# yunminjin2/KD-PointCloud

Measured on AMD Instinct MI355X. Metric: scene-flow pairs/sec fwd+bwd @ N=8192; EPE3D vs ref; 1/2/4/8 MI355X, higher is better.
Workload: dtype f32; 1 GPU; PointConvBidirection fwd+bwd+Adam (BASELINE configs[2]); model=models_bid_pointconv.PointConvBidirection, batch_per_gpu=8, global_batch=8, npoints=8192, parallelism=dp1, step=hip-graph (1 graph: fwd+bwd+flat Adam)

## Files before the change

### kd-pointcloud_amd/csrc/cost_volume.hip

```cpp
#include <algorithm>

#include "kdpc_common.h"
#include "split_bf16.h"

using namespace kdpc;
using namespace kdpc_x6;

namespace {

typedef float f32x16 __attribute__((ext_vector_type(16)));
typedef float f32x4 __attribute__((ext_vector_type(4)));

constexpr float kSlope = 0.1f;
constexpr int kRows = 32;
constexpr int kWaves = 4;

__device__ __forceinline__ float lrelu(float x) { return x > 0.f ? x : x * kSlope; }

__device__ __forceinline__ float bload(__amdgpu_buffer_rsrc_t r, unsigned off) {
  return __builtin_bit_cast(float, __builtin_amdgcn_raw_buffer_load_b32(r, (int)off, 0, 0));
}
__device__ __forceinline__ __amdgpu_buffer_rsrc_t rsrc_of(const void* p, long long bytes) {
  return __builtin_amdgcn_make_buffer_rsrc(const_cast<void*>(p), (short)0, (int)bytes, 0x00020000);
}
// ... 223 lines not shown
    bwp[ks] = split8(v);
  }
  const float w0 = wpos[cg * 3 + 0], wy = wpos[cg * 3 + 1], wz = wpos[cg * 3 + 2], bp = bpos[cg];

  const float* x1b = x1 + (long long)b * n1 * 3;
  const __amdgpu_buffer_rsrc_t x2r = rsrc_of(x2 + (long long)b * n2 * 3, (long long)n2 * 12);
  const __amdgpu_buffer_rsrc_t ixr = rsrc_of(idx + (long long)b * n1 * k, (long long)n1 * k * 4);
  const __amdgpu_buffer_rsrc_t p1r = rsrc_of(p1 + (long long)b * n1 * D_IN, (long long)n1 * D_IN * 4);
  const __amdgpu_buffer_rsrc_t p2r = rsrc_of(p2 + (long long)b * n2 * D_IN, (long long)n2 * D_IN * 4);
  const long long ob0 = (long long)b * n1 * D_OUT;
  const __amdgpu_buffer_rsrc_t outr = rsrc_of(out + ob0, (long long)n1 * D_OUT * 4);
  const __amdgpu_buffer_rsrc_t dor = rsrc_of(dout + ob0, (long long)n1 * D_OUT * 4);
  const __amdgpu_buffer_rsrc_t amr = rsrc_of(amax + ob0, (long long)n1 * D_OUT);
  const __amdgpu_buffer_rsrc_t s0r =
      rsrc_of(OVR ? slope0 + (long long)b * n1 * k * D_IN : amax, OVR ? (long long)n1 * k * D_IN : 0);
  const bool ranked = rank != nullptr;
  const __amdgpu_buffer_rsrc_t rkr = rsrc_of(ranked ? rank + (long long)b * n1 * k : idx,
                                             ranked ? (long long)n1 * k * 4 : 0);
  const long long nrow_all = (long long)nb * n1 * k;
  const __amdgpu_buffer_rsrc_t rowr = rsrc_of(rows_out, rows_out ? nrow_all * D_IN * 4 : 0);
  const __amdgpu_buffer_rsrc_t dirr = rsrc_of(dirs_out, dirs_out ? nrow_all * (ranked ? 16 : 12) : 0);
  const int nbase = b * n1;

  float gw1[DW1_MFMA ? 1 : D_OUT / 2];
  f32x16 gw[DW1_MFMA ? OT : 1];
  if constexpr (DW1_MFMA) {
#pragma unroll
    for (int t = 0; t < OT; ++t) gw[t] = f32x16{0};
  } else {
#pragma unroll
    for (int i = 0; i < D_OUT / 2; ++i) gw1[i] = 0.f;
  }
  float gb1[OT];
#pragma unroll
  for (int t = 0; t < OT; ++t) gb1[t] = 0.f;
  float gpx[2] = {0.f, 0.f}, gpy[2] = {0.f, 0.f}, gpz[2] = {0.f, 0.f};
  float gbp = 0.f;

  const int q0 = (bx * (kWaves / CS) + qw) * queries_per_wave;
  const int q1 = min(n1, q0 + queries_per_wave);
  int jn = (int)__builtin_amdgcn_raw_buffer_load_b32(ixr, (int)(((unsigned)q0 * (unsigned)k + lane) * 4u), 0, 0);
  float pv[8][2];
  float xv0, xv1, xv2, p1v, ovq[OT], dvq[OT];
  float qs0, qs1, qs2;
  auto load_q = [&](int n) {
    const int nq = min(n, n1 - 1);
    qs0 = x1b[nq * 3 + 0];
    qs1 = x1b[nq * 3 + 1];
    qs2 = x1b[nq * 3 + 2];
  };
  int amq[OT], rkn;
  auto load_idx = [&](int n) {
    jn = (int)__builtin_amdgcn_raw_buffer_load_b32(ixr, (int)(((unsigned)n * (unsigned)k + lane) * 4u), 0, 0);
  };
  auto issue = [&](int n) {
    const unsigned xo = (unsigned)jn * 12u;
    xv0 = bload(x2r, xo);
    xv1 = bload(x2r, xo + 4u);
    xv2 = bload(x2r, xo + 8u);
#pragma unroll
    for (int t = 0; t < OT; ++t) {
      const unsigned oo = (unsigned)n * D_OUT + 32 * t + l32;
      ovq[t] = bload(outr, oo * 4u);
      dvq[t] = bload(dor, oo * 4u);
      amq[t] = (int)__builtin_amdgcn_raw_buffer_load_b8(amr, (int)oo, 0, 0);
    }
    rkn = (int)__builtin_amdgcn_raw_buffer_load_b32(
        rkr, (int)(lane < k ? ((unsigned)n * (unsigned)k + lane) * 4u : kOOB), 0, 0);
    jT[lane] = jn;
    wave_lds_sync();
    load_idx(n + 1);
#pragma unroll
    for (int q = 0; q < 4; ++q) {
      const int4 j4 = *reinterpret_cast<const int4*>(jT + 8 * q + 4 * half);
      pv[2 * q][0] = bload(p2r, ((unsigned)j4.x * D_IN + cg) * 4u);
      pv[2 * q][1] = bload(p2r, ((unsigned)j4.y * D_IN + cg) * 4u);
      pv[2 * q + 1][0] = bload(p2r, ((unsigned)j4.z * D_IN + cg) * 4u);
      pv[2 * q + 1][1] = bload(p2r, ((unsigned)j4.w * D_IN + cg) * 4u);
    }
    p1v = bload(p1r, ((unsigned)n * D_IN + cg) * 4u);
  };
  float gqn[OT];
  int amn[OT], rkm = -1;
  auto tables = [&](int m, int u) {
#pragma unroll
    for (int t = 0; t < OT; ++t) {
      gqn[t] = dvq[t] * (ovq[t] > 0.f ? 1.f : kSlope);
      amn[t] = amq[t];
    }
    rkm = rkn;
    const int slot = lane < k ? (ranked ? rkm : (nbase + m) * k + lane) : -1;
    float* x = dX(u);
    x[lane] = xv0 - qs0;
    x[2 * kRows + lane] = xv1 - qs1;
    x[4 * kRows + lane] = xv2 - qs2;
    dO(u)[lane] = slot >= 0 ? (unsigned)slot * (unsigned)(D_IN * 4) : kOOB;
#pragma unroll
    for (int t = 0; t < OT; ++t) {
      gdam(u)[32 * t + l32] = make_float2(gqn[t], __int_as_float(amn[t]));
      __bf16 gh, gm, gl;
      split3(gqn[t], gh, gm, gl);
      gpl(u)[32 * t + l32] = gh;
      gpl(u)[D_OUT + 32 * t + l32] = gm;
      gpl(u)[2 * D_OUT + 32 * t + l32] = gl;
      g16(u)[32 * t + l32] = (unsigned short)amn[t];
    }
  };
  float h0[8][2];
  auto build_h0 = [&](int u) {
    const float* x = dX(u);
#pragma unroll
    for (int q = 0; q < 4; ++q) {
      const f32x4 X4 = *reinterpret_cast<const f32x4*>(x + 8 * q + 4 * half);
      const f32x4 Y4 = *reinterpret_cast<const f32x4*>(x + 2 * kRows + 8 * q + 4 * half);
      const f32x4 Z4 = *reinterpret_cast<const f32x4*>(x + 4 * kRows + 8 * q + 4 * half);
#pragma unroll
      for (int e = 0; e < 4; ++e) {
        const float pos = __fadd_rn(
            __builtin_fmaf(wz, Z4[e], __builtin_fmaf(wy, Y4[e], __fmul_rn(w0, X4[e]))), bp);
        const float z = __fadd_rn(__fadd_rn(pv[2 * q + (e >> 1)][e & 1], p1v), pos);
        h0[2 * q + (e >> 1)][e & 1] = fmaxf(z, __fmul_rn(z, kSlope));
      }
      __builtin_amdgcn_sched_barrier(0);
    }
  };
  issue(q0);
  load_q(q0);
  tables(q0, 0);
  load_q(q0 + 1);
  wave_lds_sync();
  build_h0(0);
  const int nit = CS > 1 ? queries_per_wave : q1 - q0;
  for (int it = 0; it < nit; ++it) {
    const int n = q0 + it;
    const int cu = it & 1;
    const bool act = CS == 1 || n < q1;
    float g0 = 0.f, g1 = 0.f, g2 = 0.f;
    const int rkv = rkm;
    float gq[OT];
    int amc[OT];
#pragma unroll
    for (int t = 0; t < OT; ++t) {
      gq[t] = gqn[t];
      amc[t] = amn[t];
    }
    if (act) {
      const float* xc = dX(cu);
      const unsigned* oc = dO(cu);
      const __bf16* gp = gpl(cu);
      const unsigned short* ga16 = g16(cu);
      wave_lds_sync();
      if constexpr (!DW1_MFMA) {
#pragma unroll
        for (int e = 0; e < 16; ++e) T[((e & 3) + 8 * (e >> 2) + 4 * half) * LD + l32] = h0[e >> 1][e & 1];
      }
      __builtin_amdgcn_sched_barrier(0);
      issue(n + 1);
      __builtin_amdgcn_sched_barrier(0);
      f32x16 dacc = f32x16{0};
      {
        typedef short s16x2 __attribute__((ext_vector_type(2)));
        const unsigned tgt = (unsigned)l32 * 0x00010001u;
#pragma unroll
        for (int ks = 0; ks < NKS; ++ks) {
          const int o0 = 16 * ks + 8 * half;
          const uint4 av4 = *reinterpret_cast<const uint4*>(ga16 + o0);
          const uint4 ph = *reinterpret_cast<const uint4*>(gp + o0);
          const uint4 pm = *reinterpret_cast<const uint4*>(gp + D_OUT + o0);
          const uint4 pq = *reinterpret_cast<const uint4*>(gp + 2 * D_OUT + o0);
          const unsigned aw[4] = {av4.x, av4.y, av4.z, av4.w};
          unsigned mk[4];
#pragma unroll
          for (int i = 0; i < 4; ++i) {
            const s16x2 d = __builtin_bit_cast(s16x2, aw[i] ^ tgt) - (s16x2){1, 1};
            mk[i] = __builtin_bit_cast(unsigned, d >> (s16x2){15, 15});
          }
          const uint4 mh = make_uint4(ph.x & mk[0], ph.y & mk[1], ph.z & mk[2], ph.w & mk[3]);
          const uint4 mm = make_uint4(pm.x & mk[0], pm.y & mk[1], pm.z & mk[2], pm.w & mk[3]);
          const uint4 ml = make_uint4(pq.x & mk[0], pq.y & mk[1], pq.z & mk[2], pq.w & mk[3]);
          dacc = mfma_x6(__builtin_bit_cast(bf16x8, mh), __builtin_bit_cast(bf16x8, mm),
                         __builtin_bit_cast(bf16x8, ml), bwp[ks].h, bwp[ks].m, bwp[ks].l, dacc);
          __builtin_amdgcn_sched_barrier(0);
        }
      }
      if constexpr (DW1_MFMA) {
        Planes hp[2];
#pragma unroll
        for (int ks2 = 0; ks2 < 2; ++ks2) {
          float v[8];
#pragma unroll
          for (int j = 0; j < 8; ++j) v[j] = h0[4 * ks2 + (j >> 1)][j & 1];
          hp[ks2] = split8(v);
        }
#pragma unroll
        for (int t = 0; t < OT; ++t) {
          const int am = amc[t];
          const bool mine = ((am >> 2) & 1) == half;
          const int e = (am & 3) + 4 * (am >> 3);
          __bf16 gh, gm, gl;
          split3(gq[t], gh, gm, gl);
          const unsigned sh = (e & 1) * 16;
          const unsigned bh = (unsigned)__builtin_bit_cast(unsigned short, gh) << sh;
          const unsigned bm = (unsigned)__builtin_bit_cast(unsigned short, gm) << sh;
          const unsigned bl = (unsigned)__builtin_bit_cast(unsigned short, gl) << sh;
#pragma unroll
          for (int ks2 = 0; ks2 < 2; ++ks2) {
            unsigned wh[4], wm[4], wl[4];
#pragma unroll
            for (int d = 0; d < 4; ++d) {
              const bool sel = mine && (e >> 1) == 4 * ks2 + d;
              wh[d] = sel ? bh : 0u;
              wm[d] = sel ? bm : 0u;
              wl[d] = sel ? bl : 0u;
            }
            gw[t] = mfma_x6(__builtin_bit_cast(bf16x8, make_uint4(wh[0], wh[1], wh[2], wh[3])),
                            __builtin_bit_cast(bf16x8, make_uint4(wm[0], wm[1], wm[2], wm[3])),
                            __builtin_bit_cast(bf16x8, make_uint4(wl[0], wl[1], wl[2], wl[3])),
                            hp[ks2].h, hp[ks2].m, hp[ks2].l, gw[t]);
          }
          __builtin_amdgcn_sched_barrier(0);
        }
// ... 10 lines not shown
      wave_lds_sync();
      __builtin_amdgcn_sched_barrier(0);
      float dz[8][2];
#pragma unroll
      for (int i = 0; i < 8; ++i) {
#pragma unroll
        for (int p = 0; p < 2; ++p) {
          const float d2 = dacc[2 * i + p];
          bool pass = h0[i][p] > 0.f;
          if constexpr (OVR) {
            const int e = 2 * i + p, r = (e & 3) + 8 * (e >> 2) + 4 * half;
            const unsigned o = __builtin_amdgcn_raw_buffer_load_b8(
                s0r, (int)((((unsigned)n * (unsigned)k + r) * D_IN + cg)), 0, 0);
            pass = o == 1u ? true : (o == 2u ? false : pass);
          }
          dz[i][p] = pass ? d2 : __fmul_rn(d2, kSlope);
        }
      }
      __builtin_amdgcn_sched_barrier(0);
      tables(n + 1, cu ^ 1);
      load_q(n + 2);
      __builtin_amdgcn_sched_barrier(0);
      float dpp1[2] = {0.f, 0.f};
      const unsigned cgo = (unsigned)cg * 4u;
#pragma unroll
      for (int q = 0; q < 4; ++q) {
        const uint4 O4 = *reinterpret_cast<const uint4*>(oc + 8 * q + 4 * half);
        const f32x4 X4 = *reinterpret_cast<const f32x4*>(xc + 8 * q + 4 * half);
        const f32x4 Y4 = *reinterpret_cast<const f32x4*>(xc + 2 * kRows + 8 * q + 4 * half);
        const f32x4 Z4 = *reinterpret_cast<const f32x4*>(xc + 4 * kRows + 8 * q + 4 * half);
        const unsigned o4[4] = {O4.x, O4.y, O4.z, O4.w};
#pragma unroll
        for (int i = 0; i < 4; ++i)
          __builtin_amdgcn_raw_buffer_store_b32(__float_as_uint(dz[2 * q + (i >> 1)][i & 1]), rowr,
                                                (int)(o4[i] + cgo), 0, 0);
#pragma unroll
        for (int e = 0; e < 4; ++e) {
          const float v = dz[2 * q + (e >> 1)][e & 1];
          dpp1[e & 1] = __fadd_rn(dpp1[e & 1], v);
          gpx[e & 1] = __builtin_fmaf(v, X4[e], gpx[e & 1]);
          gpy[e & 1] = __builtin_fmaf(v, Y4[e], gpy[e & 1]);
          gpz[e & 1] = __builtin_fmaf(v, Z4[e], gpz[e & 1]);
        }
        __builtin_amdgcn_sched_barrier(0);
      }
      float dp1_acc = __fadd_rn(dpp1[0], dpp1[1]);
      dp1_acc = __fadd_rn(dp1_acc, xor32(dp1_acc));
      if (half == 0) dp1[((long long)b * n1 + n) * D_IN + cg] = dp1_acc;
      gbp = __fadd_rn(gbp, dp1_acc);
#pragma unroll
      for (int e = 0; e < 16; ++e) T[((e & 3) + 8 * (e >> 2) + 4 * half) * LD + l32] = dz[e >> 1][e & 1];
      wave_lds_sync();
#pragma unroll
      for (int i = 0; i < 16; ++i) {
        const int cc = half * 16 + i;
        const float v = T[l32 * LD + cc];
        const float4 wp = wposT[hc * 32 + cc];
        g0 = __builtin_fmaf(wp.x, v, g0);
        g1 = __builtin_fmaf(wp.y, v, g1);
        g2 = __builtin_fmaf(wp.z, v, g2);
        if (i % 4 == 3) __builtin_amdgcn_sched_barrier(0);
      }
      g0 = __fadd_rn(g0, xor32(g0));
      g1 = __fadd_rn(g1, xor32(g1));
      g2 = __fadd_rn(g2, xor32(g2));
      wave_lds_sync();
    }
    if constexpr (CS > 1) {
      float4* xch = reinterpret_cast<float4*>(lds_all + XCH_AT) +
                    ((it & 1) * (kWaves / CS) + qw) * kRows;
      if (act && hc == 1 && lane < kRows) xch[lane] = make_float4(g0, g1, g2, 0.f);
      asm volatile("s_waitcnt lgkmcnt(0)\n\ts_barrier" ::: "memory");
      if (act && hc == 0) {
        const float4 o = xch[l32];
        g0 = __fadd_rn(g0, o.x);
        g1 = __fadd_rn(g1, o.y);
        g2 = __fadd_rn(g2, o.z);
      }
    }
    if (act && hc == 0) {
      const bool row = lane < k;
      if (ranked) {
        const unsigned off = (row && rkv >= 0) ? (unsigned)rkv * 16u : kOOB;
        __builtin_amdgcn_raw_buffer_store_b128(f32x4{g0, g1, g2, 0.f}, dirr, (int)off, 0, 0);
      } else {
        const unsigned off = row ? ((unsigned)((nbase + n) * k + lane)) * 12u : kOOB;
        __builtin_amdgcn_raw_buffer_store_b32(__float_as_uint(g0), dirr, (int)off, 0, 0);
        __builtin_amdgcn_raw_buffer_store_b32(__float_as_uint(g1), dirr, (int)(off == kOOB ? kOOB : off + 4u), 0, 0);
        __builtin_amdgcn_raw_buffer_store_b32(__float_as_uint(g2), dirr, (int)(off == kOOB ? kOOB : off + 8u), 0, 0);
      }
      const float s0 = sum32_lane0(row ? g0 : 0.f), s1 = sum32_lane0(row ? g1 : 0.f),
                  s2 = sum32_lane0(row ? g2 : 0.f);
      if (lane == 0) {
        float* o = dx1 + ((long long)b * n1 + n) * 3;
        o[0] = -s0;
        o[1] = -s1;
        o[2] = -s2;
      }
    }
    if (act) {
      __builtin_amdgcn_sched_barrier(0);
      asm volatile("" ::: "memory");
      build_h0((it & 1) ^ 1);
    }
  }
  float gwp0 = __fadd_rn(gpx[0], gpx[1]), gwp1 = __fadd_rn(gpy[0], gpy[1]),
        gwp2 = __fadd_rn(gpz[0], gpz[1]);
  gwp0 = __fadd_rn(gwp0, xor32(gwp0));
  gwp1 = __fadd_rn(gwp1, xor32(gwp1));
  gwp2 = __fadd_rn(gwp2, xor32(gwp2));
  __syncthreads();
  float* rw = lds_all;
  for (int w = 0; w < kWaves; ++w) {
    if (wave == w) {
      const bool first = qw == 0;
      if constexpr (DW1_MFMA) {
#pragma unroll
        for (int t = 0; t < OT; ++t)
#pragma unroll
          for (int e = 0; e < 16; ++e) {
            float* p = rw + (32 * t + (e & 3) + 8 * (e >> 2) + 4 * half) * D_IN + cg;
            *p = first ? gw[t][e] : __fadd_rn(*p, gw[t][e]);
          }
      } else {
#pragma unroll
        for (int i = 0; i < D_OUT / 2; ++i) {
          float* p = rw + (2 * i + half) * D_IN + cg;
          *p = first ? gw1[i] : __fadd_rn(*p, gw1[i]);
        }
      }
      if (hc == 0 && half == 0) {
#pragma unroll
        for (int t = 0; t < OT; ++t) {
          float* p = rw + D_OUT * D_IN + 32 * t + l32;
          *p = first ? gb1[t] : __fadd_rn(*p, gb1[t]);
        }
      }
      if (half == 0) {
        const float v4[4] = {gwp0, gwp1, gwp2, gbp};
#pragma unroll
        for (int q = 0; q < 4; ++q) {
          float* p = rw + D_OUT * D_IN + D_OUT + q * D_IN + cg;
          *p = first ? v4[q] : __fadd_rn(*p, v4[q]);
        }
      }
    }
    __syncthreads();
  }
  float* sb = slab + (long long)pblk * SLAB;
  for (int e = threadIdx.x; e < SLAB; e += blockDim.x) sb[e] = rw[e];
}

constexpr int kFwdQpw = 16;

template <int DI, int DO>
int bwd_waves_resident() {
  static const int w = [] {
    int blocks = 0, dev = 0, cus = 0;
    if (hipOccupancyMaxActiveBlocksPerMultiprocessor(&blocks,
                                                     cost_volume_bwd_kernel<DI, DO, false>,
                                                     256, 0) != hipSuccess || blocks < 1)
      blocks = 1;
    if (hipGetDevice(&dev) != hipSuccess ||
        hipDeviceGetAttribute(&cus, hipDeviceAttributeMultiprocessorCount, dev) != hipSuccess ||
        cus < 1)
      cus = 256;
    return blocks * cus * kWaves;
  }();
  return w;
}

template <int DI>
constexpr int bwd_cs() { return DI == 64 ? 2 : 1; }

template <int DI, int DO>
inline int bwd_qpw(int b, int n1) {
  const long long streams = bwd_waves_resident<DI, DO>() / bwd_cs<DI>();
  return std::max(2, (int)divupll((long long)b * n1, streams));
}

inline int bwd_qpw_of(int b, int n1, int din, int dout) {
  if (din == 32) return dout == 32 ? bwd_qpw<32, 32>(b, n1) : bwd_qpw<32, 64>(b, n1);
  return dout == 32 ? bwd_qpw<64, 32>(b, n1) : bwd_qpw<64, 64>(b, n1);
}

inline int slab_len(int din, int dout) { return dout * din + dout + 4 * din; }

template <int DI, int DO>
hipError_t fwd_launch(int b, int n1, int n2, int k, const float* x1, const float* x2,
                      const int* idx, const float* p1, const float* p2, const float* wpos,
                      const float* bpos, const float* w1, const float* b1, float* out,
                      unsigned char* amax, hipStream_t st) {
  const int gx = divup(n1, kWaves * kFwdQpw);
  dim3 grid(8 * divup(gx * b, 8));
  hipLaunchKernelGGL((cost_volume_fwd_kernel<DI, DO>), grid, dim3(256), 0, st, b, gx, n1, n2, k,
                     kFwdQpw, x1, x2, idx, p1, p2, wpos, bpos, w1, b1, out, amax);
  return hipGetLastError();
}

template <int DI, int DO>
hipError_t bwd_launch(int b, int n1, int n2, int k, const float* x1, const float* x2,
                      const int* idx, const float* p1, const float* p2, const float* wpos,
                      const float* bpos, const float* w1, const float* out,
                      const unsigned char* amax, const unsigned char* s0, const float* dout,
                      float* dp1, float* dp2_rows, float* dx1, float* ddir_rows, const int* rank,
                      float* rows, float* slab, float* dparams, hipStream_t st) {
  const int qpw = bwd_qpw<DI, DO>(b, n1);
  const int gx = divup(n1, (kWaves / bwd_cs<DI>()) * qpw);
  dim3 grid(8 * divup(gx * b, 8));
  float* rows_out = rank ? rows : dp2_rows;
  float* dirs_out = rank ? rows + (long long)b * n1 * k * DI : ddir_rows;
  if (s0)
    hipLaunchKernelGGL((cost_volume_bwd_kernel<DI, DO, true>), grid, dim3(256), 0, st, b, gx, n1,
                       n2, k, qpw, x1, x2, idx, p1, p2, wpos, bpos, w1, out, amax, s0, dout, dp1,
                       dx1, rank, rows_out, dirs_out, slab);
  else
    hipLaunchKernelGGL((cost_volume_bwd_kernel<DI, DO, false>), grid, dim3(256), 0, st, b, gx,
                       n1, n2, k, qpw, x1, x2, idx, p1, p2, wpos, bpos, w1, out, amax, s0, dout, dp1,
                       dx1, rank, rows_out, dirs_out, slab);
  hipError_t e = hipGetLastError();
  if (e != hipSuccess) return e;
  const int len = slab_len(DI, DO);
  const int nslab = gx * b;
  return colsum(nslab, len, slab, dparams, slab + (size_t)nslab * len, st);
}

__device__ __forceinline__ float4 vadd(float4 a, float4 b) {
  return make_float4(__fadd_rn(a.x, b.x), __fadd_rn(a.y, b.y), __fadd_rn(a.z, b.z),
                     __fadd_rn(a.w, b.w));
}
template <int D>
__global__ __launch_bounds__(256) void cv_rows_sum_lds_kernel(long long nkeys,
                                                              const float* __restrict__ rows,
                                                              const float* __restrict__ dirs,
                                                              const int* __restrict__ offsets,
                                                              float* __restrict__ dp2,
                                                              float* __restrict__ dx2) {
  constexpr int CH = D / 4 + 1;
  constexpr int KB = 256 / CH;
  constexpr int WR = 4096 / CH;
  __shared__ float4 win[WR * CH];
  constexpr int DQ = D / 4;
  const float4* src = reinterpret_cast<const float4*>(rows);
  const float4* srd = reinterpret_cast<const float4*>(dirs);
  const long long k0 = (long long)blockIdx.x * KB;
  const int t = threadIdx.x;
  const int kl = t / CH, ch = t - (t / CH) * CH;
  const long long key = k0 + kl;
  const bool mine = kl < KB && key < nkeys;
  const long long kend = std::min<long long>(k0 + KB, nkeys);
  const int s0 = offsets[k0], s1 = offsets[kend];
  const int j0 = mine ? offsets[key] : 0, j1 = mine ? offsets[key + 1] : 0;
  constexpr int NPT = (WR * CH + 255) / 256;
  float4 acc = make_float4(0.f, 0.f, 0.f, 0.f);
  float4 nx[NPT];
  auto fetch = [&](int w) {
    const int nr = min(WR, s1 - w);
#pragma unroll
    for (int q = 0; q < NPT; ++q) {
      const int i = t + 256 * q;
      nx[q] = i < nr * DQ ? src[(long long)w * DQ + i]
                          : (i < nr * CH ? srd[w + (i - nr * DQ)] : make_float4(0.f, 0.f, 0.f, 0.f));
    }
  };
  if (s0 < s1) fetch(s0);
  for (int w = s0; w < s1; w += WR) {
    const int nr = min(WR, s1 - w);
#pragma unroll
    for (int q = 0; q < NPT; ++q) {
      const int i = t + 256 * q;
      if (i < nr * CH)
        win[i < nr * DQ ? (i / DQ) * CH + i % DQ : (i - nr * DQ) * CH + DQ] = nx[q];
    }
    __syncthreads();
    if (w + WR < s1) fetch(w + WR);
    const int a = max(j0, w) - w, b = min(j1, w + nr) - w;
    int j = a;
    for (; j + 8 <= b; j += 8) {
      float4 v[8];
#pragma unroll
      for (int u = 0; u < 8; ++u) v[u] = win[(j + u) * CH + ch];
#pragma unroll
      for (int u = 0; u < 8; ++u) acc = vadd(acc, v[u]);
    }
    for (; j < b; ++j) acc = vadd(acc, win[j * CH + ch]);
    __syncthreads();
  }
  if (!mine) return;
  if (ch < D / 4) {
    reinterpret_cast<float4*>(dp2)[key * (D / 4) + ch] = acc;
  } else {
    float* o = dx2 + key * 3;
    o[0] = acc.x;
    o[1] = acc.y;
    o[2] = acc.z;
  }
}

template <int D>
hipError_t rows_sum_launch(long long nkeys, const float* rows, const float* dirs,
                           const int* offsets, float* dp2, float* dx2, hipStream_t st) {
  constexpr int KB = 256 / (D / 4 + 1);
  if (nkeys <= 0) return hipSuccess;
  hipLaunchKernelGGL((cv_rows_sum_lds_kernel<D>), dim3((unsigned)divupll(nkeys, KB)), dim3(256),
                     0, st, nkeys, rows, dirs, offsets, dp2, dx2);
  return hipGetLastError();
}

hipError_t rows_sum(int din, long long nkeys, const float* rows, const float* dirs,
                    const int* offsets, float* dp2, float* dx2, hipStream_t st) {
  switch (din) {
    case 32: return rows_sum_launch<32>(nkeys, rows, dirs, offsets, dp2, dx2, st);
    case 64: return rows_sum_launch<64>(nkeys, rows, dirs, offsets, dp2, dx2, st);
    case 128: return rows_sum_launch<128>(nkeys, rows, dirs, offsets, dp2, dx2, st);
    case 256: return rows_sum_launch<256>(nkeys, rows, dirs, offsets, dp2, dx2, st);
    default: return hipErrorInvalidValue;
  }
}

bool narrow(int din, int dout, int k) {
  return (din == 32 || din == 64) && (dout == 32 || dout == 64) && k >= 1 && k <= 32;
}

bool supported(int din, int dout, int k) {
  return narrow(din, dout, k) || cost_volume_wide_fused_supported(din, dout, k);
}

bool rows_fit(int b, int n1, int k, int din, int dout) {
  return !narrow(din, dout, k) || (long long)b * n1 * k * din * 4 < (1ll << 31);
}

hipError_t bwd_dispatch(int b, int n1, int n2, int k, int din, int dout, const float* x1,
                        const float* x2, const int* idx, const float* p1, const float* p2,
                        const float* wpos, const float* bpos, const float* w1, const float* out,
                        const unsigned char* amax, const unsigned char* s0,
                        const float* dout_grad, float* dp1, float* dp2_rows, float* dx1,
                        float* ddir_rows, const int* rank, float* rows, float* slab,
                        float* dparams, hipStream_t st) {
  if (!narrow(din, dout, k))
    return cost_volume_wide_fused_bwd(b, n1, n2, k, din, x1, x2, idx, p1, p2, wpos, bpos, w1, out,
                                      amax, s0, dout_grad, dp1, dp2_rows, dx1, ddir_rows, rank,
                                      rows, slab, dparams, st);
#define KDPC_CV_BWD(DI, DO)                                                                    \
  if (din == DI && dout == DO)                                                                 \
    return bwd_launch<DI, DO>(b, n1, n2, k, x1, x2, idx, p1, p2, wpos, bpos, w1, out, amax, s0,  \
                              dout_grad, dp1, dp2_rows, dx1, ddir_rows, rank, rows, slab,        \
                              dparams, st);
  KDPC_CV_BWD(32, 32)
  KDPC_CV_BWD(32, 64)
  KDPC_CV_BWD(64, 32)
  KDPC_CV_BWD(64, 64)
#undef KDPC_CV_BWD
  return hipErrorInvalidValue;
}

}

KDPC_API int kdpc_cost_volume_fwd(int b, int n1, int n2, int k, int din, int dout, const float* x1,
// ... 85 lines not shown
```

### kd-pointcloud_amd/csrc/cost_volume_wide.hip

```cpp
#include <algorithm>

#include "kdpc_common.h"
#include "split_bf16.h"

using namespace kdpc;
using namespace kdpc_x6;

namespace {

constexpr float kSlope = 0.1f;
constexpr int kBlock = 256;
constexpr int kBwdWgs = 1024;

__device__ __forceinline__ float lrelu(float x) { return x > 0.f ? x : x * kSlope; }

__global__ __launch_bounds__(kBlock) void cvw_h0_kernel(long long rows, int n1, int n2, int k,
                                                        int d, const float* __restrict__ x1,
                                                        const float* __restrict__ x2,
                                                        const int* __restrict__ idx,
                                                        const float* __restrict__ p1,
                                                        const float* __restrict__ p2,
                                                        const float* __restrict__ wpos,
                                                        const float* __restrict__ bpos,
                                                        float* __restrict__ h0) {
// ... 320 lines not shown
    bw[ks] = split8(v);
  }
  const float bias = b1[32 * w + l32];

  int jn[G::RPT], jn2[G::RPT];
  WideLoads<D> L;
  wide_load_idx<D>(s, q0, jn, rg);
  wide_load<D>(s, q0, jn, rg, c4, L);
  wide_load_idx<D>(s, q0 + 1, jn2, rg);
  __syncthreads();
  wide_build_planes<D>(L, k, rg, c4, wposT, Hp[0]);
  __syncthreads();
  for (int q = q0; q < q1; ++q) {
    const int p = (q - q0) & 1;
#pragma unroll
    for (int i = 0; i < G::RPT; ++i) jn[i] = jn2[i];
    wide_load<D>(s, q + 1 < q1 ? q + 1 : s.nq, jn, rg, c4, L);
    wide_load_idx<D>(s, q + 2 < q1 ? q + 2 : s.nq, jn2, rg);
    f32x16 acc;
#pragma unroll
    for (int e = 0; e < 16; ++e) acc[e] = 0.f;
#pragma unroll
    for (int ks = 0; ks < NKS; ++ks) {
      const int cix = l32 * (D / 8) + ((2 * ks + half) ^ (l32 & 15));
      acc = mfma_x6(Hp[p][0][cix], Hp[p][1][cix], Hp[p][2][cix], bw[ks].h, bw[ks].m, bw[ks].l, acc);
    }
    float m = -INFINITY;
    int mr = 0;
#pragma unroll
    for (int e = 0; e < 16; ++e) {
      const int row = (e & 3) + 8 * (e >> 2) + 4 * half;
      const float v = lrelu(__fadd_rn(acc[e], bias));
      if (row < k && v > m) {
        m = v;
        mr = row;
      }
    }
    const float pm = __shfl_xor(m, 32, kWave);
    const int pr = __shfl_xor(mr, 32, kWave);
    if (pm > m || (pm == m && pr < mr)) {
      m = pm;
      mr = pr;
    }
    if (half == 0) {
      out[(long long)q * D + 32 * w + l32] = m;
      amax[(long long)q * D + 32 * w + l32] = (unsigned char)mr;
    }
    if (q + 1 < q1) wide_build_planes<D>(L, k, rg, c4, wposT, Hp[p ^ 1]);
    __syncthreads();
  }
}

template <int D>
struct WideBwd {
  static constexpr int OSPLIT = D <= 128 ? 1 : 2;
  static constexpr int NKS = D / 16;
  static constexpr bool PREFETCH = D <= 128;
  static constexpr int OG = WideGeo<D>::NT / WideGeo<D>::C4;
  static constexpr int OPT = D / OG / OSPLIT;
  static constexpr int SLAB = D * D + D + 4 * D;
};

template <int D, int PART, bool OVR>
__global__ __launch_bounds__(2 * D) __attribute__((amdgpu_waves_per_eu(D == 128 ? 1 : 2))) void cvw_fused_bwd_kernel(
    int b, int n1, int n2, int k, int qpw, const float* __restrict__ x1,
    const float* __restrict__ x2, const int* __restrict__ idx, const float* __restrict__ p1,
    const float* __restrict__ p2, const float* __restrict__ wpos, const float* __restrict__ bpos,
    const float* __restrict__ w1, const bf16x8* __restrict__ w1p, const float* __restrict__ out,
    const unsigned char* __restrict__ amax, const unsigned char* __restrict__ slope0,
    const float* __restrict__ dout,
    float* __restrict__ dp1, float* __restrict__ dp2_rows, float* __restrict__ dx1,
    float* __restrict__ ddir_rows, const int* __restrict__ rank, float* __restrict__ rows,
    float* __restrict__ slab) {
  using G = WideGeo<D>;
  using W = WideBwd<D>;
  constexpr int NG2 = G::NT / 32;
  constexpr int CPG = D / NG2;
  constexpr bool MAIN = PART != 2, DW1 = PART != 1;
  __shared__ __attribute__((aligned(16))) float Hs[2][32 * G::LD];
  __shared__ __attribute__((aligned(16))) float4 dirs[2][32];
  __shared__ __attribute__((aligned(16))) float2 gam[2][D];
  __shared__ __attribute__((aligned(16))) __bf16 gpl[2][3][D];
  __shared__ __attribute__((aligned(16))) unsigned short gam16[2][D];
  __shared__ __attribute__((aligned(16))) float4 red[G::RG][G::C4];
  __shared__ __attribute__((aligned(16))) float4 red2[NG2][32];
  __shared__ __attribute__((aligned(16))) float4 wposT[D];
  const int t = threadIdx.x, lane = t & 63, w = t >> 6, half = lane >> 5, l32 = lane & 31;
  const int c4 = t % G::C4, rg = t / G::C4;
  const WideSrc s = wide_src<D>(b, n1, n2, k, x1, x2, idx, p1, p2);
  const int q0 = blockIdx.x * qpw;
  const int q1 = min(s.nq, q0 + qpw);
  float* sb = slab + (long long)blockIdx.x * W::SLAB;
  const int obase = DW1 ? (int)blockIdx.y * (D / W::OSPLIT) : 0;
  if (q0 >= q1) {
    for (int e = t; e < W::SLAB; e += G::NT) {
      const bool dw = e < D * D ? (e / D - obase >= 0 && e / D - obase < D / W::OSPLIT)
                                : (e < D * D + D && blockIdx.y == 0);
      if (dw ? DW1 : (MAIN && e >= D * D + D)) sb[e] = 0.f;
    }
    return;
  }
  const __amdgpu_buffer_rsrc_t outr = rsrc_of(out, (long long)s.nq * D * 4);
  const __amdgpu_buffer_rsrc_t dor = rsrc_of(dout, (long long)s.nq * D * 4);
  const __amdgpu_buffer_rsrc_t amr = rsrc_of(amax, (long long)s.nq * D);
  const __amdgpu_buffer_rsrc_t s0r = rsrc_of(OVR ? slope0 : amax, OVR ? (long long)s.nq * k * D : 0);
  const bool ranked = rank != nullptr;
  const __amdgpu_buffer_rsrc_t rkr = rsrc_of(ranked ? rank : idx, ranked ? (long long)s.nq * k * 4 : 0);
  wide_consts<D>(wpos, bpos, wposT);
  const bf16x8* w1row = w1p + (long long)(w * W::NKS * 3) * 64 + lane;
  float4 gw[DW1 ? W::OPT : 1];
#pragma unroll
  for (int i = 0; i < (DW1 ? W::OPT : 1); ++i) gw[i] = make_float4(0.f, 0.f, 0.f, 0.f);
  float gb1 = 0.f;
  float4 gwp[3], gbp = make_float4(0.f, 0.f, 0.f, 0.f);
#pragma unroll
  for (int j = 0; j < 3; ++j) gwp[j] = make_float4(0.f, 0.f, 0.f, 0.f);

  float ov = 0.f, dv = 0.f;
  unsigned av = 0;
  auto load_out = [&](int q) {
    const bool ok = q < s.nq && t < D;
    const unsigned oo = (unsigned)q * D + t;
    ov = bld(outr, ok ? oo * 4u : kOOB);
    dv = bld(dor, ok ? oo * 4u : kOOB);
    av = __builtin_amdgcn_raw_buffer_load_b8(amr, (int)(ok ? oo : kOOB), 0, 0);
  };
  int rk[G::RPT], rkd = -1;
  auto load_rank = [&](int q) {
#pragma unroll
    for (int i = 0; i < G::RPT; ++i) {
      const int r = rg + G::RG * i;
      rk[i] = (int)__builtin_amdgcn_raw_buffer_load_b32(
          rkr, (int)(r < k ? ((unsigned)q * (unsigned)k + r) * 4u : kOOB), 0, 0);
    }
    rkd = (int)__builtin_amdgcn_raw_buffer_load_b32(
        rkr, (int)(l32 < k ? ((unsigned)q * (unsigned)k + l32) * 4u : kOOB), 0, 0);
  };
  auto stage_out = [&](int p) {
    if (t < D) {
      const float g = ov > 0.f ? dv : dv * kSlope;
      gam[p][t] = make_float2(g, __int_as_float((int)av));
      __bf16 gh, gm, gl;
      split3(g, gh, gm, gl);
      gpl[p][0][t] = gh;
      gpl[p][1][t] = gm;
      gpl[p][2][t] = gl;
      gam16[p][t] = (unsigned short)av;
    }
  };

  int jn[G::RPT], jn2[G::RPT];
  WideLoads<D> L;
  wide_load_idx<D>(s, q0, jn, rg);
  wide_load<D>(s, q0, jn, rg, c4, L);
  load_out(q0);
  wide_load_idx<D>(s, q0 + 1, jn2, rg);
  __syncthreads();
  wide_build<D>(L, k, rg, c4, wposT, Hs[0], dirs[0]);
  stage_out(0);
  __syncthreads();
  for (int q = q0; q < q1; ++q) {
    const int p = (q - q0) & 1;
    const bool more = q + 1 < q1;
    if (MAIN && ranked) load_rank(q);
    auto next_loads = [&]() {
#pragma unroll
      for (int i = 0; i < G::RPT; ++i) jn[i] = jn2[i];
      wide_load<D>(s, more ? q + 1 : s.nq, jn, rg, c4, L);
      load_out(more ? q + 1 : s.nq);
      wide_load_idx<D>(s, q + 2 < q1 ? q + 2 : s.nq, jn2, rg);
    };
    if constexpr (W::PREFETCH) next_loads();
    float* H = Hs[p];
    const float2* ga = gam[p];
    f32x16 dacc;
    if constexpr (MAIN) {
#pragma unroll
    for (int e = 0; e < 16; ++e) dacc[e] = 0.f;
    constexpr int PF = 2;
    Planes bq[PF];
    auto bload = [&](int ks, Planes& bb) {
      bb.h = w1row[(3 * ks + 0) * 64];
      bb.m = w1row[(3 * ks + 1) * 64];
      bb.l = w1row[(3 * ks + 2) * 64];
    };
#pragma unroll
    for (int i = 0; i < PF; ++i) bload(i, bq[i]);
    typedef short s16x2 __attribute__((ext_vector_type(2)));
    const unsigned tgt = (unsigned)l32 * 0x00010001u;
#pragma unroll 2
    for (int ks = 0; ks < W::NKS; ++ks) {
      const int o0 = 16 * ks + 8 * half;
      const uint4 av4 = *reinterpret_cast<const uint4*>(&gam16[p][o0]);
      const uint4 ph = *reinterpret_cast<const uint4*>(&gpl[p][0][o0]);
      const uint4 pm = *reinterpret_cast<const uint4*>(&gpl[p][1][o0]);
      const uint4 pl = *reinterpret_cast<const uint4*>(&gpl[p][2][o0]);
      const unsigned aw[4] = {av4.x, av4.y, av4.z, av4.w};
      unsigned mk[4];
#pragma unroll
      for (int i = 0; i < 4; ++i) {
        const s16x2 d = __builtin_bit_cast(s16x2, aw[i] ^ tgt) - (s16x2){1, 1};
        mk[i] = __builtin_bit_cast(unsigned, d >> (s16x2){15, 15});
      }
      const uint4 mh = make_uint4(ph.x & mk[0], ph.y & mk[1], ph.z & mk[2], ph.w & mk[3]);
      const uint4 mm = make_uint4(pm.x & mk[0], pm.y & mk[1], pm.z & mk[2], pm.w & mk[3]);
      const uint4 ml = make_uint4(pl.x & mk[0], pl.y & mk[1], pl.z & mk[2], pl.w & mk[3]);
      dacc = mfma_x6(__builtin_bit_cast(bf16x8, mh), __builtin_bit_cast(bf16x8, mm),
                     __builtin_bit_cast(bf16x8, ml), bq[ks % PF].h, bq[ks % PF].m, bq[ks % PF].l,
                     dacc);
      if (ks + PF < W::NKS) bload(ks + PF, bq[ks % PF]);
      __builtin_amdgcn_sched_barrier(0);
    }
    }
    if constexpr (DW1) {
#pragma unroll
    for (int i = 0; i < W::OPT; ++i) {
      const float2 g = ga[obase + rg * W::OPT + i];
      const float4 hv = *reinterpret_cast<const float4*>(H + __float_as_int(g.y) * G::LD + 4 * c4);
      gw[i].x = __builtin_fmaf(g.x, hv.x, gw[i].x);
      gw[i].y = __builtin_fmaf(g.x, hv.y, gw[i].y);
      gw[i].z = __builtin_fmaf(g.x, hv.z, gw[i].z);
      gw[i].w = __builtin_fmaf(g.x, hv.w, gw[i].w);
      if (i % 4 == 3) __builtin_amdgcn_sched_barrier(0);
    }
    if (t < D && blockIdx.y == 0) gb1 = __fadd_rn(gb1, ga[t].x);
    }
    __syncthreads();
    if constexpr (MAIN) {
#pragma unroll
    for (int e = 0; e < 16; ++e) {
      const int row = (e & 3) + 8 * (e >> 2) + 4 * half;
      const int a = row * G::LD + 32 * w + l32;
      const float hv = H[a];
      float sl = hv > 0.f ? 1.f : kSlope;
      if constexpr (OVR) {
        const unsigned o = __builtin_amdgcn_raw_buffer_load_b8(
            s0r, (int)(((unsigned)q * (unsigned)k + row) * D + 32 * w + l32), 0, 0);
        sl = o == 1u ? 1.f : (o == 2u ? kSlope : sl);
      }
      H[a] = dacc[e] * sl;
    }
    __syncthreads();
    {
      float4 sp = make_float4(0.f, 0.f, 0.f, 0.f);
      float* d2 = dp2_rows + (long long)q * k * D + 4 * c4;
#pragma unroll
      for (int i = 0; i < G::RPT; ++i) {
        const int r = rg + G::RG * i;
        const float4 v = *reinterpret_cast<const float4*>(H + r * G::LD + 4 * c4);
        const float4 dr = dirs[p][r];
        if (ranked) {
          if (r < k && rk[i] >= 0) *reinterpret_cast<float4*>(rows + (long long)rk[i] * D + 4 * c4) = v;
        } else if (r < k && dp2_rows) {
          *reinterpret_cast<float4*>(d2 + (long long)r * D) = v;
        }
        sp.x = __fadd_rn(sp.x, v.x);
        sp.y = __fadd_rn(sp.y, v.y);
        sp.z = __fadd_rn(sp.z, v.z);
        sp.w = __fadd_rn(sp.w, v.w);
        const float dd[3] = {dr.x, dr.y, dr.z};
#pragma unroll
        for (int j = 0; j < 3; ++j) {
          gwp[j].x = __builtin_fmaf(v.x, dd[j], gwp[j].x);
          gwp[j].y = __builtin_fmaf(v.y, dd[j], gwp[j].y);
          gwp[j].z = __builtin_fmaf(v.z, dd[j], gwp[j].z);
          gwp[j].w = __builtin_fmaf(v.w, dd[j], gwp[j].w);
        }
      }
      red[rg][c4] = sp;
    }
    {
      const int r = t & 31, g2 = t >> 5;
      float a0 = 0.f, a1 = 0.f, a2 = 0.f;
#pragma unroll 4
      for (int i = 0; i < CPG / 4; ++i) {
        const int c = g2 * CPG + 4 * i;
        const float4 v = *reinterpret_cast<const float4*>(H + r * G::LD + c);
        const float vv[4] = {v.x, v.y, v.z, v.w};
#pragma unroll
        for (int e = 0; e < 4; ++e) {
          const float4 wq = wposT[c + e];
          a0 = __builtin_fmaf(wq.x, vv[e], a0);
          a1 = __builtin_fmaf(wq.y, vv[e], a1);
          a2 = __builtin_fmaf(wq.z, vv[e], a2);
        }
      }
      red2[g2][r] = make_float4(a0, a1, a2, 0.f);
    }
    }
    if constexpr (!W::PREFETCH) next_loads();
    if (more) {
      wide_build<D>(L, k, rg, c4, wposT, Hs[p ^ 1], dirs[p ^ 1]);
      stage_out(p ^ 1);
    }
    __syncthreads();
    if (MAIN && rg == 0) {
      float4 v = red[0][c4];
#pragma unroll
      for (int g = 1; g < G::RG; ++g) {
        const float4 x = red[g][c4];
        v.x = __fadd_rn(v.x, x.x);
        v.y = __fadd_rn(v.y, x.y);
        v.z = __fadd_rn(v.z, x.z);
        v.w = __fadd_rn(v.w, x.w);
      }
      *reinterpret_cast<float4*>(dp1 + (long long)q * D + 4 * c4) = v;
      gbp.x = __fadd_rn(gbp.x, v.x);
      gbp.y = __fadd_rn(gbp.y, v.y);
      gbp.z = __fadd_rn(gbp.z, v.z);
      gbp.w = __fadd_rn(gbp.w, v.w);
    }
    if (MAIN && w == G::NW - 1 && half == 0) {
      float4 v = red2[0][l32];
#pragma unroll
      for (int g = 1; g < NG2; ++g) {
        const float4 x = red2[g][l32];
        v.x = __fadd_rn(v.x, x.x);
        v.y = __fadd_rn(v.y, x.y);
        v.z = __fadd_rn(v.z, x.z);
      }
      const bool row = l32 < k;
      if (row && ranked) {
        if (rkd >= 0)
          *reinterpret_cast<float4*>(rows + (long long)b * n1 * k * D + (long long)rkd * 4) =
              make_float4(v.x, v.y, v.z, 0.f);
      } else if (row && ddir_rows) {
        float* dd = ddir_rows + ((long long)q * k + l32) * 3;
        dd[0] = v.x;
        dd[1] = v.y;
        dd[2] = v.z;
      }
      float s0 = row ? v.x : 0.f, s1 = row ? v.y : 0.f, s2 = row ? v.z : 0.f;
#pragma unroll
      for (int m = 16; m >= 1; m >>= 1) {
        s0 = __fadd_rn(s0, __shfl_xor(s0, m, kWave));
        s1 = __fadd_rn(s1, __shfl_xor(s1, m, kWave));
        s2 = __fadd_rn(s2, __shfl_xor(s2, m, kWave));
      }
      if (l32 == 0) {
        float* o = dx1 + (long long)q * 3;
        o[0] = -s0;
        o[1] = -s1;
        o[2] = -s2;
      }
    }
  }
  if constexpr (DW1) {
#pragma unroll
    for (int i = 0; i < W::OPT; ++i)
      *reinterpret_cast<float4*>(sb + (long long)(obase + rg * W::OPT + i) * D + 4 * c4) = gw[i];
    if (t < D && blockIdx.y == 0) sb[D * D + t] = gb1;
  }
  if constexpr (!MAIN) return;
  __syncthreads();
  float4* fold = reinterpret_cast<float4*>(&Hs[0][0]);
#pragma unroll
  for (int j = 0; j < 3; ++j) fold[(rg * 3 + j) * G::C4 + c4] = gwp[j];
  __syncthreads();
  if (rg == 0) {
#pragma unroll
    for (int j = 0; j < 3; ++j) {
      float4 v = fold[j * G::C4 + c4];
      for (int g = 1; g < G::RG; ++g) {
        const float4 x = fold[(g * 3 + j) * G::C4 + c4];
        v.x = __fadd_rn(v.x, x.x);
        v.y = __fadd_rn(v.y, x.y);
        v.z = __fadd_rn(v.z, x.z);
        v.w = __fadd_rn(v.w, x.w);
      }
      *reinterpret_cast<float4*>(sb + D * D + D + j * D + 4 * c4) = v;
    }
    *reinterpret_cast<float4*>(sb + D * D + 4 * D + 4 * c4) = gbp;
  }
}

__global__ __launch_bounds__(256) void cvw_w1_planes_kernel(int d, const float* __restrict__ w1,
                                                            bf16x8* __restrict__ w1p) {
  const int e = blockIdx.x * 256 + threadIdx.x;
  const int nks = d / 16;
  if (e >= (d / 32) * nks * 64) return;
  const int lane = e & 63, q = e >> 6, ks = q % nks, w = q / nks;
  float v[8];
#pragma unroll
  for (int j = 0; j < 8; ++j) v[j] = w1[(16 * ks + 8 * (lane >> 5) + j) * d + 32 * w + (lane & 31)];
  const Planes pl = split8(v);
  bf16x8* dst = w1p + (long long)q * 3 * 64 + lane;
  dst[0] = pl.h;
  dst[64] = pl.m;
  dst[128] = pl.l;
}

inline int fused_qpw(long long nq, int d, bool bwd) {
  const int target = bwd || d == 256 ? 256 : 512;
  return (int)std::max<long long>(2, divupll(nq, target));
}

}

namespace kdpc {

bool cost_volume_wide_fused_supported(int din, int dout, int k) {
  return din == dout && (din == 128 || din == 256) && k >= 1 && k <= 32;
}

hipError_t cost_volume_wide_fused_fwd(int b, int n1, int n2, int k, int d, const float* x1,
                                      const float* x2, const int* idx, const float* p1,
                                      const float* p2, const float* wpos, const float* bpos,
                                      const float* w1, const float* b1, float* out,
// ... 147 lines not shown
```

### kd-pointcloud_amd/csrc/kdpc_common.h

```cpp
#pragma once
#include <hip/hip_runtime.h>
#include <stdint.h>

#include "kdpc.h"

#define KDPC_API extern "C" __attribute__((visibility("default")))

namespace kdpc {

constexpr int kWave = 64;

__host__ __device__ inline int divup(int a, int b) { return (a + b - 1) / b; }
__host__ __device__ inline long long divupll(long long a, long long b) { return (a + b - 1) / b; }

__device__ __forceinline__ float dist3(float x1, float y1, float z1, float x2, float y2,
                                       float z2) {
  const float dx = x2 - x1, dy = y2 - y1, dz = z2 - z1;
  return __builtin_fmaf(dz, dz, __builtin_fmaf(dy, dy, __fmul_rn(dx, dx)));
}

__device__ __forceinline__ float sqnorm3(float x, float y, float z) {
  return __fadd_rn(__fadd_rn(__fmul_rn(x, x), __fmul_rn(y, y)), __fmul_rn(z, z));
}
__device__ __forceinline__ float sqdist_expanded(float qx, float qy, float qz, float sq, float rx,
                                                 float ry, float rz, float sr) {
  const float dot = __builtin_fmaf(qz, rz, __builtin_fmaf(qy, ry, __fmul_rn(qx, rx)));
  return __fadd_rn(__fadd_rn(-2.0f * dot, sq), sr);
}

__device__ __forceinline__ int lane_id() { return threadIdx.x & (kWave - 1); }

__device__ __forceinline__ void wave_lds_sync() {
  asm volatile("" ::: "memory");
  __builtin_amdgcn_wave_barrier();
  asm volatile("" ::: "memory");
}

__device__ __forceinline__ unsigned wave_max_u32(unsigned v) {
#pragma unroll
  for (int o = 32; o >= 1; o >>= 1) {
    unsigned w = __shfl_xor(v, o, kWave);
    v = w > v ? w : v;
  }
  return v;
}
__device__ __forceinline__ unsigned wave_min_u32(unsigned v) {
#pragma unroll
  for (int o = 32; o >= 1; o >>= 1) {
    unsigned w = __shfl_xor(v, o, kWave);
    v = w < v ? w : v;
  }
  return v;
}

__device__ __forceinline__ float wave_shr1(float v, float fill) {
  return __int_as_float(__builtin_amdgcn_update_dpp(__float_as_int(fill), __float_as_int(v),
                                                    0x138, 0xf, 0xf, false));
}
__device__ __forceinline__ int wave_shr1(int v, int fill) {
  return __builtin_amdgcn_update_dpp(fill, v, 0x138, 0xf, 0xf, false);
}

__device__ __forceinline__ unsigned long long lanemask_lt() {
  const int l = lane_id();
  return l == 0 ? 0ull : (~0ull >> (64 - l));
}

size_t colsum_scratch_floats(int nrows, long long len);
hipError_t colsum(int nrows, long long len, const float* slab, float* dst, float* scratch,
                  hipStream_t st);

bool cost_volume_wide_fused_supported(int din, int dout, int k);
hipError_t cost_volume_wide_fused_fwd(int b, int n1, int n2, int k, int d, const float* x1,
                                      const float* x2, const int* idx, const float* p1,
                                      const float* p2, const float* wpos, const float* bpos,
                                      const float* w1, const float* b1, float* out,
                                      unsigned char* amax, hipStream_t st);
size_t cost_volume_wide_fused_bwd_workspace_floats(int b, int n1, int d);
hipError_t cost_volume_wide_fused_bwd(int b, int n1, int n2, int k, int d, const float* x1,
                                      const float* x2, const int* idx, const float* p1,
                                      const float* p2, const float* wpos, const float* bpos,
                                      const float* w1, const float* out,
                                      const unsigned char* amax, const unsigned char* slope0,
                                      const float* dout, float* dp1, float* dp2_rows, float* dx1,
                                      float* ddir_rows, const int* rank, float* rows, float* ws,
                                      float* dparams, hipStream_t st);

}

#define KDPC_CHECK_ARG(cond)                       \
  do {                                             \
    if (!(cond)) return (int)hipErrorInvalidValue; \
  } while (0)

#define KDPC_RETURN_LAUNCH() return (int)hipGetLastError()
```

Measured before the change: 589.4 pairs/s.

## Skip dead neighbor rows in cost-volume backward via argmax liveness flags

Computes a per-query bitmask of which neighbor rows were ever selected by the max-pool argmax. That mask is used to skip writing gradient rows for dead neighbors, and a liveness flag is stored in the previously unused fourth lane of the direction record. The row-sum kernel reads these flags first and skips loading dead rows, and it halves its LDS window while prefetching flags two windows ahead. This cuts global memory traffic in the backward gather, at the cost of extra flag loads and cross-lane reductions, and it depends on the flag and row layout staying consistent across kernels.

Result: faster. 602.0 pairs/s, median of 6 (+2.1%).

```diff
diff --git a/kd-pointcloud_amd/csrc/cost_volume.hip b/kd-pointcloud_amd/csrc/cost_volume.hip
--- a/kd-pointcloud_amd/csrc/cost_volume.hip
+++ b/kd-pointcloud_amd/csrc/cost_volume.hip
@@ -329,14 +329,19 @@
   };
   float gqn[OT];
   int amn[OT], rkm = -1;
+  unsigned livem = 0u;
   auto tables = [&](int m, int u) {
+    unsigned lv = 0u;
 #pragma unroll
     for (int t = 0; t < OT; ++t) {
       gqn[t] = dvq[t] * (ovq[t] > 0.f ? 1.f : kSlope);
       amn[t] = amq[t];
-    }
+      lv |= 1u << (amn[t] & 31);
+    }
+    livem = wave_or_u32(lv);
     rkm = rkn;
-    const int slot = lane < k ? (ranked ? rkm : (nbase + m) * k + lane) : -1;
+    const bool keep = !ranked || ((livem >> (lane & 31)) & 1u);
+    const int slot = lane < k && keep ? (ranked ? rkm : (nbase + m) * k + lane) : -1;
     float* x = dX(u);
     x[lane] = xv0 - qs0;
     x[2 * kRows + lane] = xv1 - qs1;
@@ -384,6 +389,7 @@
     const bool act = CS == 1 || n < q1;
     float g0 = 0.f, g1 = 0.f, g2 = 0.f;
     const int rkv = rkm;
+    const unsigned lvv = livem;
     float gq[OT];
     int amc[OT];
 #pragma unroll
@@ -560,7 +566,8 @@
       const bool row = lane < k;
       if (ranked) {
         const unsigned off = (row && rkv >= 0) ? (unsigned)rkv * 16u : kOOB;
-        __builtin_amdgcn_raw_buffer_store_b128(f32x4{g0, g1, g2, 0.f}, dirr, (int)off, 0, 0);
+        const float fl = (lvv >> (lane & 31)) & 1u ? 1.f : 0.f;
+        __builtin_amdgcn_raw_buffer_store_b128(f32x4{g0, g1, g2, fl}, dirr, (int)off, 0, 0);
       } else {
         const unsigned off = row ? ((unsigned)((nbase + n) * k + lane)) * 12u : kOOB;
         __builtin_amdgcn_raw_buffer_store_b32(__float_as_uint(g0), dirr, (int)off, 0, 0);
@@ -716,42 +723,73 @@
                                                               float* __restrict__ dx2) {
   constexpr int CH = D / 4 + 1;
   constexpr int KB = 256 / CH;
-  constexpr int WR = 4096 / CH;
+  constexpr int WF4 = 2048;
+  constexpr int WR = WF4 / CH;
   __shared__ float4 win[WR * CH];
   constexpr int DQ = D / 4;
-  const float4* src = reinterpret_cast<const float4*>(rows);
-  const float4* srd = reinterpret_cast<const float4*>(dirs);
   const long long k0 = (long long)blockIdx.x * KB;
   const int t = threadIdx.x;
   const int kl = t / CH, ch = t - (t / CH) * CH;
   const long long key = k0 + kl;
   const bool mine = kl < KB && key < nkeys;
   const long long kend = std::min<long long>(k0 + KB, nkeys);
-  const int s0 = offsets[k0], s1 = offsets[kend];
+  const int s0 = __builtin_amdgcn_readfirstlane(offsets[k0]);
+  const int s1 = __builtin_amdgcn_readfirstlane(offsets[kend]);
   const int j0 = mine ? offsets[key] : 0, j1 = mine ? offsets[key + 1] : 0;
-  constexpr int NPT = (WR * CH + 255) / 256;
+  constexpr int NPT = (WR * DQ + 255) / 256;
+  constexpr int NDT = (WR + 255) / 256;
   float4 acc = make_float4(0.f, 0.f, 0.f, 0.f);
-  float4 nx[NPT];
-  auto fetch = [&](int w) {
-    const int nr = min(WR, s1 - w);
+  float4 nx[NPT], nd[NDT];
+  float fl[NPT];
+  auto ld4 = [](__amdgpu_buffer_rsrc_t r, unsigned off) {
+    const auto v = __builtin_amdgcn_raw_buffer_load_b128(r, (int)off, 0, 0);
+    return make_float4(__uint_as_float(v[0]), __uint_as_float(v[1]), __uint_as_float(v[2]),
+                       __uint_as_float(v[3]));
+  };
+  auto flags = [&](int w) {
+    const int nr = min(WR, s1 - min(w, s1));
+    const __amdgpu_buffer_rsrc_t dr = rsrc_of(dirs + (long long)w * 4, (long long)nr * 16);
 #pragma unroll
     for (int q = 0; q < NPT; ++q) {
       const int i = t + 256 * q;
-      nx[q] = i < nr * DQ ? src[(long long)w * DQ + i]
-                          : (i < nr * CH ? srd[w + (i - nr * DQ)] : make_float4(0.f, 0.f, 0.f, 0.f));
-    }
-  };
-  if (s0 < s1) fetch(s0);
+      fl[q] = bload(dr, i < nr * DQ ? (unsigned)(i / DQ) * 16u + 12u : kOOB);
+    }
+  };
+  auto fetch = [&](int w) {
+    const int nr = min(WR, s1 - min(w, s1));
+    const __amdgpu_buffer_rsrc_t rr = rsrc_of(rows + (long long)w * D, (long long)nr * D * 4);
+    const __amdgpu_buffer_rsrc_t dr = rsrc_of(dirs + (long long)w * 4, (long long)nr * 16);
+#pragma unroll
+    for (int q = 0; q < NPT; ++q) {
+      const int i = t + 256 * q;
+      nx[q] = ld4(rr, i < nr * DQ && fl[q] != 0.f ? (unsigned)i * 16u : kOOB);
+    }
+#pragma unroll
+    for (int q = 0; q < NDT; ++q) {
+      const int i = t + 256 * q;
+      nd[q] = ld4(dr, i < nr ? (unsigned)i * 16u : kOOB);
+    }
+  };
+  if (s0 < s1) {
+    flags(s0);
+    fetch(s0);
+    flags(s0 + WR);
+  }
   for (int w = s0; w < s1; w += WR) {
     const int nr = min(WR, s1 - w);
 #pragma unroll
     for (int q = 0; q < NPT; ++q) {
       const int i = t + 256 * q;
-      if (i < nr * CH)
-        win[i < nr * DQ ? (i / DQ) * CH + i % DQ : (i - nr * DQ) * CH + DQ] = nx[q];
+      if (i < nr * DQ) win[(i / DQ) * CH + i % DQ] = nx[q];
+    }
+#pragma unroll
+    for (int q = 0; q < NDT; ++q) {
+      const int i = t + 256 * q;
+      if (i < nr) win[i * CH + DQ] = nd[q];
     }
     __syncthreads();
-    if (w + WR < s1) fetch(w + WR);
+    fetch(w + WR);
+    flags(w + 2 * WR);
     const int a = max(j0, w) - w, b = min(j1, w + nr) - w;
     int j = a;
     for (; j + 8 <= b; j += 8) {
diff --git a/kd-pointcloud_amd/csrc/cost_volume_wide.hip b/kd-pointcloud_amd/csrc/cost_volume_wide.hip
--- a/kd-pointcloud_amd/csrc/cost_volume_wide.hip
+++ b/kd-pointcloud_amd/csrc/cost_volume_wide.hip
@@ -426,6 +426,7 @@
   __shared__ __attribute__((aligned(16))) float2 gam[2][D];
   __shared__ __attribute__((aligned(16))) __bf16 gpl[2][3][D];
   __shared__ __attribute__((aligned(16))) unsigned short gam16[2][D];
+  __shared__ unsigned livew[2][D / 64];
   __shared__ __attribute__((aligned(16))) float4 red[G::RG][G::C4];
   __shared__ __attribute__((aligned(16))) float4 red2[NG2][32];
   __shared__ __attribute__((aligned(16))) float4 wposT[D];
@@ -490,6 +491,8 @@
       gpl[p][1][t] = gm;
       gpl[p][2][t] = gl;
       gam16[p][t] = (unsigned short)av;
+      const unsigned lv = wave_or_u32(1u << (av & 31u));
+      if (lane == 0) livew[p][w] = lv;
     }
   };
 
@@ -517,6 +520,7 @@
     if constexpr (W::PREFETCH) next_loads();
     float* H = Hs[p];
     const float2* ga = gam[p];
+    unsigned live = 0u;
     f32x16 dacc;
     if constexpr (MAIN) {
 #pragma unroll
@@ -588,13 +592,19 @@
     {
       float4 sp = make_float4(0.f, 0.f, 0.f, 0.f);
       float* d2 = dp2_rows + (long long)q * k * D + 4 * c4;
+      if (ranked) {
+        live = livew[p][0];
+#pragma unroll
+        for (int i = 1; i < D / 64; ++i) live |= livew[p][i];
+      }
 #pragma unroll
       for (int i = 0; i < G::RPT; ++i) {
         const int r = rg + G::RG * i;
         const float4 v = *reinterpret_cast<const float4*>(H + r * G::LD + 4 * c4);
         const float4 dr = dirs[p][r];
         if (ranked) {
-          if (r < k && rk[i] >= 0) *reinterpret_cast<float4*>(rows + (long long)rk[i] * D + 4 * c4) = v;
+          if (r < k && rk[i] >= 0 && ((live >> r) & 1u))
+            *reinterpret_cast<float4*>(rows + (long long)rk[i] * D + 4 * c4) = v;
         } else if (r < k && dp2_rows) {
           *reinterpret_cast<float4*>(d2 + (long long)r * D) = v;
         }
@@ -667,7 +677,7 @@
       if (row && ranked) {
         if (rkd >= 0)
           *reinterpret_cast<float4*>(rows + (long long)b * n1 * k * D + (long long)rkd * 4) =
-              make_float4(v.x, v.y, v.z, 0.f);
+              make_float4(v.x, v.y, v.z, (live >> l32) & 1u ? 1.f : 0.f);
       } else if (row && ddir_rows) {
         float* dd = ddir_rows + ((long long)q * k + l32) * 3;
         dd[0] = v.x;
diff --git a/kd-pointcloud_amd/csrc/kdpc_common.h b/kd-pointcloud_amd/csrc/kdpc_common.h
--- a/kd-pointcloud_amd/csrc/kdpc_common.h
+++ b/kd-pointcloud_amd/csrc/kdpc_common.h
@@ -53,6 +53,20 @@
   return v;
 }
 
+template <int CTRL>
+__device__ __forceinline__ unsigned or_dpp(unsigned v) {
+  return v | (unsigned)__builtin_amdgcn_update_dpp(0, (int)v, CTRL, 0xf, 0xf, false);
+}
+__device__ __forceinline__ unsigned wave_or_u32(unsigned v) {
+  v = or_dpp<0xB1>(v);
+  v = or_dpp<0x4E>(v);
+  v = or_dpp<0x141>(v);
+  v = or_dpp<0x140>(v);
+  const int s = (int)v;
+  return (unsigned)(__builtin_amdgcn_readlane(s, 0) | __builtin_amdgcn_readlane(s, 16) |
+                    __builtin_amdgcn_readlane(s, 32) | __builtin_amdgcn_readlane(s, 48));
+}
+
 __device__ __forceinline__ float wave_shr1(float v, float fill) {
   return __int_as_float(__builtin_amdgcn_update_dpp(__float_as_int(fill), __float_as_int(v),
                                                     0x138, 0xf, 0xf, false));
```
